# 92MING/Stable-Renderer

Hardware: AMD Instinct MI355X
Metric: frames/sec @512^2, SD1.5 20-step img2img, 8-view overlap (higher is better)
Workload: dtype f16

## Files before the change

### stable-renderer_amd/csrc/igemm.hip

```cpp
#include "sr_common.h"
#ifndef SR_IGEMM_TRACE
#define SR_IGEMM_TRACE 0
#endif
#if SR_IGEMM_TRACE
#define SR_TS(k) do { if (threadIdx.x == 0) ts_[k] = wall_clock64(); } while (0)
#else
#define SR_TS(k) do { } while (0)
#endif
#include <stdlib.h>
#include <type_traits>

namespace {

#define SR_FOLD(p) ((p).row_stats != nullptr || (p).ln_inline != 0)
__device__ __forceinline__ float2 sr_fold_stat(const sr_igemm_args& p, const int m, const int m0) {
  extern __shared__ __attribute__((aligned(16))) char sr_lds_front[];
  if (p.ln_inline) return *(const float2*)(sr_lds_front + 8 * (m - m0));
  return *(const float2*)(p.row_stats + 2 * (int64_t)m);
}

template <typename T, int BM, int BN, int WAVES_M, int WAVES_N, int LDS_AVAIL, bool GEGLU, int VCAP, bool VECPRE>
__device__ __forceinline__ void epilogue_rows_h(const sr_igemm_args& p, f32x4 (&acc)[BN / WAVES_N / 16][BM / WAVES_M / 16], char* smem, const int M,
                                                const int rpb, const int m0, const int n0, const int pm0, const int qn0, const int wv,
                                                const int lane) {
  constexpr int NW = WAVES_M * WAVES_N, TM = BM / WAVES_M / 16, TN = BN / WAVES_N / 16;
  constexpr int WCOLS = BN / WAVES_N, OCOLS = GEGLU ? WCOLS / 2 : WCOLS;
  constexpr int ROWB = OCOLS * 2 + 16;
  constexpr int CPR = OCOLS * 2 / 16, RPI = 64 / CPR;
  constexpr int VEC_B = 2 * BN * 4;
  constexpr int LDS_ROWS = VECPRE ? LDS_AVAIL : LDS_AVAIL - VEC_B;
  constexpr int ACC = TM * TN * 4;
  constexpr auto iters = [](int tmp) { return (tmp * 16 + RPI - 1) / RPI; };
  constexpr auto fits = [](int tmp) { return tmp >= 1 && TM % tmp == 0 && NW * tmp * 16 * ROWB <= LDS_ROWS; };
  constexpr auto pre_ok = [](int tmp) { return ACC + (TM / tmp) * ((tmp * 16 + RPI - 1) / RPI) * 4 + 48 <= VCAP; };
  constexpr auto roll_ok = [](int tmp) { return TM / tmp > 1 && ACC + 2 * ((tmp * 16 + RPI - 1) / RPI) * 4 + 40 <= VCAP; };
  constexpr int T_LDS = fits(TM) ? TM : (fits(TM / 2) ? TM / 2 : 1);
  constexpr int TMP = pre_ok(T_LDS) ? T_LDS : (roll_ok(T_LDS) ? T_LDS : ((T_LDS > 1 && roll_ok(T_LDS / 2) && fits(T_LDS / 2)) ? T_LDS / 2 : ((T_LDS > 1 && roll_ok(1)) ? 1 : T_LDS)));
  constexpr int ROWS = TMP * 16, ITER = iters(TMP), NPASS = TM / TMP;
  constexpr bool PRE = pre_ok(TMP);
  constexpr bool ROLL = !PRE && roll_ok(TMP);
  static_assert(OCOLS % 8 == 0 && NW * 16 * ROWB <= LDS_ROWS, "epilogue staging");
  const int c16 = lane & 15, g4 = lane >> 4;
  const float scale = p.scale;
  const int N = p.N;
  const int ldr = p.rowvec_ld ? p.rowvec_ld : N;
  const int ldo = GEGLU ? (N >> 1) : N;
  float* lvec = (float*)(VECPRE ? smem - VEC_B : smem);
  char* wl = smem + (VECPRE ? 0 : VEC_B) + wv * (ROWS * ROWB);
  const int lr = lane / CPR, lc = lane - lr * CPR;
  const int ncol = (GEGLU ? ((n0 + qn0) >> 1) : (n0 + qn0)) + lc * 8;
  const bool lane_on = lr < RPI && ncol < ldo;
  const int tid = wv * 64 + lane;

  float4 vb = make_float4(0.f, 0.f, 0.f, 0.f), vc = make_float4(0.f, 0.f, 0.f, 0.f);
  if constexpr (!VECPRE) {
    const bool vec_lane = tid < BN / 4 && n0 + tid * 4 < N;
    if (vec_lane) {
      if (p.bias) vb = *(const float4*)(p.bias + n0 + tid * 4);
      if (SR_FOLD(p)) vc = *(const float4*)(p.colsum + n0 + tid * 4);
    }
  }
  uint4 resid[PRE ? NPASS * ITER : 1];
  if constexpr (PRE) {
    if (p.residual) {
#pragma unroll
      for (int ps = 0; ps < NPASS; ++ps)
#pragma unroll
        for (int it = 0; it < ITER; ++it) {
          const int row = it * RPI + lr, m = m0 + pm0 + ps * ROWS + row;
          resid[ps * ITER + it] = make_uint4(0, 0, 0, 0);
          if (lane_on && row < ROWS && m < M) resid[ps * ITER + it] = *(const uint4*)((const _Float16*)p.residual + (int64_t)m * ldo + ncol);
        }
    }
  }
  uint4 rcur[ROLL ? ITER : 1], rnext[ROLL ? ITER : 1];
  auto roll_load = [&](uint4 (&dst)[ROLL ? ITER : 1], int ps) {
#pragma unroll
    for (int it = 0; it < (ROLL ? ITER : 1); ++it) {
      const int row = it * RPI + lr, m = m0 + pm0 + ps * ROWS + row;
      dst[it] = make_uint4(0, 0, 0, 0);
      if (lane_on && row < ROWS && m < M) dst[it] = *(const uint4*)((const _Float16*)p.residual + (int64_t)m * ldo + ncol);
    }
  };
  if constexpr (ROLL) { if (p.residual) roll_load(rcur, 0); }
  __syncthreads();
  if constexpr (!VECPRE) {
    if (tid < BN / 4) { *(float4*)(lvec + tid * 4) = vb; *(float4*)(lvec + BN + tid * 4) = vc; }
    __syncthreads();
  }
#pragma unroll
  for (int ps = 0; ps < NPASS; ++ps) {
#pragma unroll
    for (int t = 0; t < TMP; ++t) {
      const int tm = ps * TMP + t;
      const int m = m0 + pm0 + tm * 16 + c16;
      const int b = (p.rowvec && m < M) ? m / rpb : 0;
      float2 rs = make_float2(1.f, 0.f);
      if (SR_FOLD(p) && m < M) rs = sr_fold_stat(p, m, m0);
#pragma unroll
      for (int tn = 0; tn < TN; ++tn) {
        const int nl = qn0 + tn * 16 + 4 * g4, n = n0 + nl;
        float v[4] = {acc[tn][tm][0] * scale, acc[tn][tm][1] * scale, acc[tn][tm][2] * scale, acc[tn][tm][3] * scale};
        if (n < N) {
          if (SR_FOLD(p)) {
            const float4 cs = *(const float4*)(lvec + BN + nl);
            v[0] = fmaf(rs.x, v[0], rs.y * cs.x); v[1] = fmaf(rs.x, v[1], rs.y * cs.y);
            v[2] = fmaf(rs.x, v[2], rs.y * cs.z); v[3] = fmaf(rs.x, v[3], rs.y * cs.w);
          }
          if (p.bias) { const float4 bv = *(const float4*)(lvec + nl); v[0] += bv.x; v[1] += bv.y; v[2] += bv.z; v[3] += bv.w; }
          if (p.rowvec) { const float4 rv = *(const float4*)(p.rowvec + (int64_t)b * ldr + n); v[0] += rv.x; v[1] += rv.y; v[2] += rv.z; v[3] += rv.w; }
        }
        if (p.act == 1) { for (int r = 0; r < 4; ++r) v[r] = sr_silu_f(v[r]); }
        else if (p.act == 3) { for (int r = 0; r < 4; ++r) v[r] = sr_gelu_f(v[r]); }
        else if (p.act == 4) { for (int r = 0; r < 4; ++r) v[r] = fminf(fmaxf((v[r] + 1.0f) * 0.5f, 0.0f), 1.0f); }
        char* dst = wl + (t * 16 + c16) * ROWB;
        if constexpr (GEGLU) {
          const float o0 = v[0] * sr_gelu_f(v[1]), o1 = v[2] * sr_gelu_f(v[3]);
          h16x2 hv = {(_Float16)o0, (_Float16)o1};
          *(h16x2*)(dst + (tn * 8 + 2 * g4) * 2) = hv;
        } else {
          h16x4 hv = {(_Float16)v[0], (_Float16)v[1], (_Float16)v[2], (_Float16)v[3]};
          *(h16x4*)(dst + (tn * 16 + 4 * g4) * 2) = hv;
        }
      }
    }
    __builtin_amdgcn_s_waitcnt(0xC07F);
    __builtin_amdgcn_wave_barrier();
    if constexpr (ROLL) { if (p.residual && ps + 1 < NPASS) roll_load(rnext, ps + 1); }
#pragma unroll
    for (int it = 0; it < ITER; ++it) {
      const int row = it * RPI + lr, m = m0 + pm0 + ps * ROWS + row;
      if (!(lane_on && row < ROWS && m < M)) continue;
      uint4 raw = *(const uint4*)(wl + row * ROWB + lc * 16);
      const int64_t oi = (int64_t)m * ldo + ncol;
      if (p.residual) {
        const h16x8 rr = PRE ? __builtin_bit_cast(h16x8, resid[PRE ? ps * ITER + it : 0])
                       : ROLL ? __builtin_bit_cast(h16x8, rcur[ROLL ? it : 0]) : *(const h16x8*)((const _Float16*)p.residual + oi);
        h16x8 hv = __builtin_bit_cast(h16x8, raw);
#pragma unroll
        for (int e = 0; e < 8; ++e) hv[e] = (_Float16)((float)hv[e] + (float)rr[e]);
        raw = __builtin_bit_cast(uint4, hv);
      }
      *(uint4*)((_Float16*)p.out + oi) = raw;
    }
    if constexpr (ROLL) {
#pragma unroll
      for (int it = 0; it < ITER; ++it) rcur[it] = rnext[it];
    }
    __builtin_amdgcn_wave_barrier();
  }
}

template <typename T, int BM, int BN, int WAVES_M, int WAVES_N, int LDS_AVAIL, bool BLOCK_SYNC = true, int VCAP = 256, bool VECPRE = false>
__device__ __forceinline__ void epilogue_rows(const sr_igemm_args& p, f32x4 (&acc)[BN / WAVES_N / 16][BM / WAVES_M / 16], char* smem, const int M,
                                              const int rpb, const int m0, const int n0, const int pm0, const int qn0, const int wv,
                                              const int lane) {
  constexpr int NW = WAVES_M * WAVES_N, TM = BM / WAVES_M / 16, TN = BN / WAVES_N / 16;
  const int c16 = lane & 15, g4 = lane >> 4;
  const float scale = p.scale;
  const int N = p.N;
  const int ldr = p.rowvec_ld ? p.rowvec_ld : N;
  {
    const int ldo = (p.act == 2) ? (N >> 1) : N;
    const bool o32 = p.out_f32 || sizeof(T) == 4;
    const int oes = o32 ? 4 : 2;
    if constexpr (sizeof(T) == 2) {
      if (!o32 && (ldo * 2) % 16 == 0) {
        static_assert(BLOCK_SYNC, "the fp16 epilogue synchronises the workgroup itself");
        if (p.act == 2) epilogue_rows_h<T, BM, BN, WAVES_M, WAVES_N, LDS_AVAIL, true, VCAP, VECPRE>(p, acc, smem, M, rpb, m0, n0, pm0, qn0, wv, lane);
        else            epilogue_rows_h<T, BM, BN, WAVES_M, WAVES_N, LDS_AVAIL, false, VCAP, VECPRE>(p, acc, smem, M, rpb, m0, n0, pm0, qn0, wv, lane);
        return;
      }
    }
    if ((ldo * oes) % 16 == 0) {
      constexpr int WCOLS = BN / WAVES_N;
      constexpr int TMP = (NW * (BM / WAVES_M) * (WCOLS * 4 + 16) <= LDS_AVAIL) ? TM : 1;
      const int ocols = (p.act == 2) ? WCOLS / 2 : WCOLS;
      const int rowb = ocols * oes + 16;
      if constexpr (BLOCK_SYNC) __syncthreads();
      char* wl = smem + wv * ((TMP * 16) * rowb);
      const int cpr = ocols * oes / 16;
      const int rpi = 64 / cpr;
      const int lr = lane / cpr, lc = lane - lr * cpr;
      const int ncol0 = (p.act == 2) ? ((n0 + qn0) >> 1) : (n0 + qn0);
      const int epc_o = 16 / oes;
#pragma unroll
     for (int tm0 = 0; tm0 < TM; tm0 += TMP) {
#pragma unroll
      for (int tm = tm0; tm < tm0 + TMP; ++tm) {
        const int m = m0 + pm0 + tm * 16 + c16;
        const int b = (m < M) ? m / rpb : 0;
        float2 rs = make_float2(1.f, 0.f);
        if (SR_FOLD(p) && m < M) rs = sr_fold_stat(p, m, m0);
#pragma unroll
        for (int tn = 0; tn < TN; ++tn) {
          const int n = n0 + qn0 + tn * 16 + 4 * g4;
          float v[4] = {acc[tn][tm][0] * scale, acc[tn][tm][1] * scale, acc[tn][tm][2] * scale, acc[tn][tm][3] * scale};
          if (n < N) {
            if (SR_FOLD(p)) {
              const float4 cs = *(const float4*)(p.colsum + n);
              v[0] = fmaf(rs.x, v[0], rs.y * cs.x); v[1] = fmaf(rs.x, v[1], rs.y * cs.y);
              v[2] = fmaf(rs.x, v[2], rs.y * cs.z); v[3] = fmaf(rs.x, v[3], rs.y * cs.w);
            }
            if (p.bias) { const float4 bv = *(const float4*)(p.bias + n); v[0] += bv.x; v[1] += bv.y; v[2] += bv.z; v[3] += bv.w; }
            if (p.rowvec) { const float4 rv = *(const float4*)(p.rowvec + (int64_t)b * ldr + n); v[0] += rv.x; v[1] += rv.y; v[2] += rv.z; v[3] += rv.w; }
          }
          if (p.act == 1) { for (int r = 0; r < 4; ++r) v[r] = sr_silu_f(v[r]); }
          else if (p.act == 3) { for (int r = 0; r < 4; ++r) v[r] = sr_gelu_f(v[r]); }
          else if (p.act == 4) { for (int r = 0; r < 4; ++r) v[r] = fminf(fmaxf((v[r] + 1.0f) * 0.5f, 0.0f), 1.0f); }
          char* dst = wl + ((tm - tm0) * 16 + c16) * rowb;
          if (p.act == 2) {
            const float o0 = v[0] * sr_gelu_f(v[1]), o1 = v[2] * sr_gelu_f(v[3]);
            const int col = tn * 8 + 2 * g4;
            if (o32) *(float2*)(dst + col * 4) = make_float2(o0, o1);
            else { h16x2 hv = {(_Float16)o0, (_Float16)o1}; *(h16x2*)(dst + col * 2) = hv; }
          } else {
            const int col = tn * 16 + 4 * g4;
            if (o32) *(float4*)(dst + col * 4) = make_float4(v[0], v[1], v[2], v[3]);
            else { h16x4 hv = {(_Float16)v[0], (_Float16)v[1], (_Float16)v[2], (_Float16)v[3]}; *(h16x4*)(dst + col * 2) = hv; }
          }
        }
      }
      __builtin_amdgcn_s_waitcnt(0xC07F);
      __builtin_amdgcn_wave_barrier();
      for (int r0 = 0; r0 < TMP * 16; r0 += rpi) {
        const int row = r0 + lr;
        if (lr >= rpi || row >= TMP * 16) continue;
        const int m = m0 + pm0 + tm0 * 16 + row, ncol = ncol0 + lc * epc_o;
        if (m >= M || ncol >= ldo) continue;
        uint4 raw = *(const uint4*)(wl + row * rowb + lc * 16);
        const int64_t oi = (int64_t)m * ldo + ncol;
        if (p.residual) {
          if constexpr (sizeof(T) == 2) {
            if (o32) {
              float4 f = __builtin_bit_cast(float4, raw);
              const h16x4 r4 = *(const h16x4*)((const _Float16*)p.residual + oi);
              f.x += (float)r4[0]; f.y += (float)r4[1]; f.z += (float)r4[2]; f.w += (float)r4[3];
              raw = __builtin_bit_cast(uint4, f);
            } else {
              const h16x8 rr = *(const h16x8*)((const _Float16*)p.residual + oi);
              h16x8 hv = __builtin_bit_cast(h16x8, raw);
#pragma unroll
              for (int e = 0; e < 8; ++e) hv[e] = (_Float16)((float)hv[e] + (float)rr[e]);
              raw = __builtin_bit_cast(uint4, hv);
            }
          } else {
            float4 f = __builtin_bit_cast(float4, raw);
            const float4 rr = *(const float4*)((const float*)p.residual + oi);
            f.x += rr.x; f.y += rr.y; f.z += rr.z; f.w += rr.w;
            raw = __builtin_bit_cast(uint4, f);
          }
        }
        *(uint4*)((char*)p.out + oi * oes) = raw;
      }
      __builtin_amdgcn_wave_barrier();
     }
      return;
    }
#pragma unroll
    for (int tm = 0; tm < TM; ++tm) {
      const int m = m0 + pm0 + tm * 16 + c16;
      if (m >= M) continue;
      const int b = m / rpb;
#pragma unroll
      for (int tn = 0; tn < TN; ++tn) {
        const int n = n0 + qn0 + tn * 16 + 4 * g4;
        if (n >= N) continue;
        float v[4] = {acc[tn][tm][0] * scale, acc[tn][tm][1] * scale, acc[tn][tm][2] * scale, acc[tn][tm][3] * scale};
        const int nv = (N - n) < 4 ? (N - n) : 4;
        if (SR_FOLD(p)) {
          const float2 rs = sr_fold_stat(p, m, m0);
          for (int r = 0; r < nv; ++r) v[r] = fmaf(rs.x, v[r], rs.y * p.colsum[n + r]);
        }
        if (p.bias) { for (int r = 0; r < nv; ++r) v[r] += p.bias[n + r]; }
        if (p.rowvec) { for (int r = 0; r < nv; ++r) v[r] += p.rowvec[(int64_t)b * ldr + n + r]; }
        if (p.act == 1) { for (int r = 0; r < 4; ++r) v[r] = sr_silu_f(v[r]); }
        else if (p.act == 3) { for (int r = 0; r < 4; ++r) v[r] = sr_gelu_f(v[r]); }
        else if (p.act == 4) { for (int r = 0; r < 4; ++r) v[r] = fminf(fmaxf((v[r] + 1.0f) * 0.5f, 0.0f), 1.0f); }
        if (p.act == 2) {
          float o0 = v[0] * sr_gelu_f(v[1]), o1 = v[2] * sr_gelu_f(v[3]);
          const int64_t oi = (int64_t)m * ldo + (n >> 1);
          if (p.residual) { o0 += sr_load_f((const T*)p.residual + oi); o1 += sr_load_f((const T*)p.residual + oi + 1); }
          if (p.out_f32) { float* o = (float*)p.out + oi; o[0] = o0; o[1] = o1; }
          else { T* o = (T*)p.out + oi; sr_store_f(o, o0); sr_store_f(o + 1, o1); }
// ... 568 lines not shown
  if (ntail > SR_IGEMM_SPLIT_COUNTERS) as.split_counters = nullptr;
  hipLaunchKernelGGL(ks, dim3(ntail, S), dim3(256), lds, st, as, M, Ho, Wo, NTv, ntail, tile0);
  if (!as.split_counters) {
    constexpr int FR = (BM / 32) * (BN / 32);
    hipLaunchKernelGGL((splitk_reduce_kernel<T, BM, BN>), dim3(ntail * FR), dim3(256), 0, st, a, M, Ho * Wo, S, NTv, ntail, tile0);
  }
  SR_CHECK_LAUNCH("sr_igemm(split-K)");
  return SR_OK;
}

__global__ __launch_bounds__(512, 1) void conv3p_kernel(const sr_igemm_args p, const int M, const int NT, const int nwg) {
  using T = _Float16;
  extern __shared__ __attribute__((aligned(16))) char smem_all[];
  char* const smem = smem_all + 8 * 256;
  constexpr int BM = 256, BN = 320, WAVES_M = 4, WAVES_N = 2, TM = 4, TN = 10;
  constexpr int APITCH = 80, ABYTES = 32768, BBYTES = BN * 64, BOFF = 2 * ABYTES, LDS_TOTAL = BOFF + 4 * BBYTES;
  const int tid = threadIdx.x, lane = tid & 63;
  const int wv = __builtin_amdgcn_readfirstlane(tid >> 6);
  if (p.prefetch)
    sr_prefetch_touch(p.prefetch, p.prefetch_bytes, (int64_t)blockIdx.x * 512 + tid, (int64_t)gridDim.x * 512,
                      __builtin_amdgcn_readfirstlane(sr_lds_addr(smem_all) + wv * 256));
  const int wg = sr_xcd_remap(blockIdx.x, nwg);
  const int mt = wg / NT, nt = wg - mt * NT;
  const int m0 = mt * BM, n0 = nt * BN;
  const int H = p.H, W = p.W, C1 = p.C1, rpb = H * W;
  const int ipt = rpb >= 256 ? 1 : 256 / rpb;
  const int Ri = rpb >= 256 ? 256 / W : H;
  const int PW = W + 2, HPI = (Ri + 2) * PW, HR = ipt * HPI;
  const int b0 = m0 / rpb, y0 = (m0 - b0 * rpb) / W;

  unsigned aoffg[4];
#pragma unroll
  for (int i = 0; i < 4; ++i) {
    const int u = (wv * 4 + i) * 64 + lane;
    const int hrow = u / 5, ch = u - hrow * 5;
    const int img = hrow / HPI, rem = hrow - img * HPI, hr = rem / PW, hc = rem - hr * PW;
    const int y = y0 + hr - 1, x = hc - 1, b = b0 + img;
    const bool ok = ch < 4 && hrow < HR && y >= 0 && y < H && x >= 0 && x < W && b < p.B;
    aoffg[i] = ok ? (unsigned)(((((int64_t)b * H + y) * W + x) * C1) * 2 + ch * 16) : 0xFFFFFFFFu;
    if (!ok) {
      *(uint4*)(smem + (wv * 4 + i) * 1024 + lane * 16) = make_uint4(0, 0, 0, 0);
      *(uint4*)(smem + ABYTES + (wv * 4 + i) * 1024 + lane * 16) = make_uint4(0, 0, 0, 0);
    }
  }
  asm volatile("s_waitcnt lgkmcnt(0)" ::: "memory");
  const int lrow = lane >> 2;
  const int lchunk = (0x1320 >> (4 * ((lane & 3) ^ ((lrow >> 2) & 3)))) & 3;
  const unsigned wlane = (unsigned)(lrow * 9 * C1 * 2 + lchunk * 16);
  const unsigned ldsA = __builtin_amdgcn_readfirstlane(sr_lds_addr(smem)), ldsB = ldsA + BOFF;
  int ac = 0;
  auto issueA = [&](int buf, int i) {
    if (aoffg[i] != 0xFFFFFFFFu) sr_glds16_asm_saddr(aoffg[i], (const char*)p.a + (int64_t)ac * 64, ldsA + buf * ABYTES + (wv * 4 + i) * 1024);
  };
  int lc = 0, lt = 0;
  auto issueB = [&](int slot) {
    const char* wb = (const char*)p.w + ((int64_t)n0 * 9 * C1 + lt * C1 + lc * 32) * 2;
#pragma unroll
    for (int i = 0; i < 3; ++i) {
      const int gi = (i * 8 + wv) < 20 ? (i * 8 + wv) : 19;
      sr_glds16_asm_saddr(wlane, wb + (int64_t)gi * 16 * 9 * C1 * 2, ldsB + slot * BBYTES + gi * 1024);
    }
    if (++lt == 9) { lt = 0; ++lc; }
  };

  const int c16 = lane & 15, g4 = lane >> 4;
  const int wm = wv >> 1, wn = wv & 1;
  const int pm0 = wm * 64, qn0 = wn * 160;
  int aoff0, adel[TM];
  {
    const int riw = Ri * W;
    auto hrow_of = [&](int pi) { const int img = pi / riw, q = pi - img * riw, r = q / W, cx = q - r * W; return img * HPI + r * PW + cx; };
    aoff0 = hrow_of(pm0 + c16) * APITCH + g4 * 16;
#pragma unroll
    for (int j = 0; j < TM; ++j) adel[j] = __builtin_amdgcn_readfirstlane((hrow_of(pm0 + j * 16) - hrow_of(pm0)) * APITCH);
  }
  const int foffB = qn0 * 64 + c16 * 64 + ((((c16 >> 2) & 3) ^ ((0x2130 >> (4 * g4)) & 3)) << 4);
  const int pw80 = PW * APITCH;

  f32x4 acc[TN][TM];
#pragma unroll
  for (int a = 0; a < TN; ++a)
#pragma unroll
    for (int b = 0; b < TM; ++b) acc[a][b] = f32x4{0.f, 0.f, 0.f, 0.f};

  const int NC = C1 / 32;
  {
    const unsigned m0k = sr_m0_save();
#pragma unroll
    for (int i = 0; i < 4; ++i) issueA(0, i);
    ac = 1;
    issueB(0); issueB(1); issueB(2);
    sr_m0_restore(m0k);
  }
  int s = 0;
  auto chunk = [&](auto lastc, const int c) {
    constexpr bool LASTC = decltype(lastc)::value;
    auto step = [&](auto tc) {
      constexpr int t = decltype(tc)::value;
      constexpr int nx = LASTC ? (t <= 6 ? 6 : (t == 7 ? 3 : 0))
                               : 6 + (t >= 1 && t <= 4) + (t >= 2 && t <= 5) + (t >= 3 && t <= 6);
      asm volatile("s_waitcnt vmcnt(%0)" ::"n"(nx) : "memory");
      __builtin_amdgcn_s_barrier();
      const char* Bq = smem + BOFF + (s & 3) * BBYTES + foffB;
      int to = (t / 3) * pw80 + (t % 3) * APITCH + (c & 1) * ABYTES;
      asm volatile("" : "+s"(to));
      uint4 xf[TM], wf[TN];
#pragma unroll
      for (int j = 0; j < TM; ++j) xf[j] = *(const uint4*)(smem + aoff0 + (adel[j] + to));
#pragma unroll
      for (int tn = 0; tn < TN; ++tn) wf[tn] = *(const uint4*)(Bq + tn * 1024);
      if (!LASTC || t < 6) {
        const unsigned m0k = sr_m0_save();
        issueB((s + 3) & 3);
        if constexpr (!LASTC) { if (t < 4) issueA((c + 1) & 1, t); if (t == 3) ++ac; }
        sr_m0_restore(m0k);
      }
#pragma unroll
      for (int tn = 0; tn < TN; ++tn)
#pragma unroll
        for (int tm = 0; tm < TM; ++tm) sr_mma(acc[tn][tm], wf[tn], xf[tm], T());
      ++s;
    };
    step(std::integral_constant<int, 0>{}); step(std::integral_constant<int, 1>{}); step(std::integral_constant<int, 2>{});
    step(std::integral_constant<int, 3>{}); step(std::integral_constant<int, 4>{}); step(std::integral_constant<int, 5>{});
    step(std::integral_constant<int, 6>{}); step(std::integral_constant<int, 7>{}); step(std::integral_constant<int, 8>{});
  };
  for (int c = 0; c < NC - 1; ++c) chunk(std::false_type{}, c);
  chunk(std::true_type{}, NC - 1);

  epilogue_rows<T, BM, BN, WAVES_M, WAVES_N, LDS_TOTAL>(p, acc, smem, M, rpb, m0, n0, pm0, qn0, wv, lane);
}

static bool conv3p_ok(const sr_igemm_args& a, int M) {
  if (a.dtype != SR_F16 || a.KH != 3 || a.stride != 1 || a.upsample || a.C2 || a.transpose_out || a.row_stats || a.ln_inline || a.pad_br) return false;
  if (a.C1 % 64 || a.N % 320 || M % 256 || a.act == 2) return false;
  const int rpb = a.H * a.W;
  if (a.W < 8 || 256 % a.W) { if (!(rpb < 256 && 256 % rpb == 0)) return false; }
  if (rpb >= 256 ? (rpb % 256 != 0 || 256 % a.W != 0) : (256 % rpb != 0)) return false;
  const int ipt = rpb >= 256 ? 1 : 256 / rpb, Ri = rpb >= 256 ? 256 / a.W : a.H;
  if ((int64_t)a.B * rpb * a.C1 * 2 >= 0xFFFFFFFFLL) return false;
  return ipt * (Ri + 2) * (a.W + 2) * 80 <= 32768;
}

static int launch_conv3p(const sr_igemm_args& a, int M, hipStream_t st) {
  constexpr int lds = 2 * 32768 + 4 * 320 * 64 + 8 * 256;
  const int NT = a.N / 320, nwg = (M / 256) * NT;
  static bool attr_set = false;
  if (!attr_set) { (void)hipFuncSetAttribute((const void*)conv3p_kernel, hipFuncAttributeMaxDynamicSharedMemorySize, lds); attr_set = true; }
  hipLaunchKernelGGL(conv3p_kernel, dim3(nwg), dim3(512), lds, st, a, M, NT, nwg);
  SR_CHECK_LAUNCH("sr_igemm(conv3p)");
  return SR_OK;
}

static inline int plan_split(int64_t tiles, int KT, int slots, double t_k, int64_t tile_ws_bytes, int64_t ws_bytes, int* tile0, int forceS = 0) {
  const int64_t full = tiles / slots, tail = tiles - full * slots;
  *tile0 = (int)(full * slots);
  if (tail == 0) return 1;
  if (forceS > 0)
    return (KT / forceS >= 4 && (int64_t)forceS * tail * tile_ws_bytes <= ws_bytes) ? forceS : -1;
  if (const char* fs = getenv("SR_SPLIT_S")) {
    const int S = atoi(fs);
    if (S >= 1 && KT / S >= 4 && (int64_t)S * tail * tile_ws_bytes <= ws_bytes) return S;
  }
  double best = (double)KT * t_k;
  int bestS = 1;
  for (int S = 2; S <= 16; ++S) {
    if (KT / S < 8 || (int64_t)S * tail * tile_ws_bytes > ws_bytes) break;
    const int64_t rounds = (tail * S + slots - 1) / slots;
    const double t = (double)rounds * ((KT + S - 1) / S) * t_k + (double)(2 * S * tail * tile_ws_bytes) / 4.0e6 + 14.0;
    if (t < best * 0.9) { best = t; bestS = S; }
  }
  return bestS;
}

template <typename T, bool TRANS>
int dispatch(const sr_igemm_args& a, int M, int Ho, int Wo, hipStream_t st) {
  const int n128 = (a.N + 127) / 128, n64 = (a.N + 63) / 64;
  const int64_t wg_128x128 = (int64_t)((M + 127) / 128) * n128;
  const bool waste128 = (n128 * 128 - a.N) * 8 > a.N;
  const char* fenv = getenv("SR_IGEMM_TILE");
  const int force = fenv ? atoi(fenv) : a.tile;
  static const bool split_off = getenv("SR_SPLITK") && atoi(getenv("SR_SPLITK")) == 0;
  const int KT = a.KH * a.KH * ((a.C1 + a.C2) / (int)(128 / sizeof(T)));
  const int forceS = a.split > 1 ? a.split : 0;
  const bool can_split = !TRANS && !split_off && a.split >= 0 && a.workspace && a.act != 2 && a.N % 4 == 0 && !a.ln_inline;
  const bool may_split = can_split && KT >= 32;
  const bool deep_split = can_split && KT >= 8 && (force == 14 || force == 15);
  if (forceS && !((may_split && (force == 2 || force == 3)) || deep_split))
    SR_FAIL(SR_ERR_INVALID, "sr_igemm: split = %d needs tile 2 / 3 (K >= 32 steps) or 14 / 15 (K >= 8 steps), a workspace, no GEGLU / transposed output", a.split);
  if constexpr (!TRANS) {
    if (deep_split && forceS) {
      int tile0 = 0;
      const int64_t tiles = force == 15 ? wg_128x128 : (int64_t)((M + 127) / 128) * n64;
      const int S = plan_split(tiles, KT, 256, 1.0, 128 * (force == 15 ? 128 : 64) * 4, a.workspace_bytes, &tile0, forceS);
      if (S < 0) SR_FAIL(SR_ERR_INVALID, "sr_igemm: split = %d does not fit this shape (K steps %d, workspace %lld B)", a.split, KT, (long long)a.workspace_bytes);
      if (S > 1) return force == 15 ? launch_split<T, 128, 128, 4>(a, M, Ho, Wo, tile0, S, st) : launch_split<T, 128, 64, 6>(a, M, Ho, Wo, tile0, S, st);
      SR_FAIL(SR_ERR_INVALID, "sr_igemm: split = %d: nothing to split (whole rounds of workgroups only)", a.split);
    }
    if (may_split && (force == 2 || force == 3)) {
      int tile0 = 0;
      if (force == 2) {
        const int S = plan_split(wg_128x128, KT, 512, 1.2, 128 * 128 * 4, a.workspace_bytes, &tile0, forceS);
        if (S < 0) SR_FAIL(SR_ERR_INVALID, "sr_igemm: split = %d does not fit this shape (K steps %d, workspace %lld B)", a.split, KT, (long long)a.workspace_bytes);
        if (S > 1) return launch_split<T, 128, 128>(a, M, Ho, Wo, tile0, S, st);
      } else {
        const int S = plan_split((int64_t)((M + 127) / 128) * n64, KT, 768, 0.93, 128 * 64 * 4, a.workspace_bytes, &tile0, forceS);
        if (S < 0) SR_FAIL(SR_ERR_INVALID, "sr_igemm: split = %d does not fit this shape (K steps %d, workspace %lld B)", a.split, KT, (long long)a.workspace_bytes);
        if (S > 1) return launch_split<T, 128, 64>(a, M, Ho, Wo, tile0, S, st);
      }
      if (forceS) SR_FAIL(SR_ERR_INVALID, "sr_igemm: split = %d: nothing to split (whole rounds of workgroups only)", a.split);
    }
  }
  if (force == 2) return launch_ln<T, 128, 128, 2, 2, 2, TRANS>(a, M, Ho, Wo, st);
  if (force == 3) return launch_ln<T, 128, 64, 2, 2, 2, TRANS>(a, M, Ho, Wo, st);
  if (force == 4) return launch_ln<T, 64, 64, 2, 2, 2, TRANS>(a, M, Ho, Wo, st);
  if (force == 13) return launch_ln<T, 64, 64, 2, 2, 8, TRANS>(a, M, Ho, Wo, st);
  if (force == 14) return launch_ln<T, 128, 64, 2, 2, 6, TRANS>(a, M, Ho, Wo, st);
  if (force == 15) return launch_ln<T, 128, 128, 2, 2, 4, TRANS>(a, M, Ho, Wo, st);
  if (force == 8) {
    if constexpr (!TRANS && sizeof(T) == 2) { if (conv3p_ok(a, M)) return launch_conv3p(a, M, st); }
    SR_FAIL(SR_ERR_INVALID, "sr_igemm: tile 8 (patch-stationary 3x3) needs fp16, KH=3, stride 1, one source, N %% 320 == 0, "
                            "256-pixel tiles of whole rows / images (H=%d W=%d M=%d N=%d)", a.H, a.W, M, a.N);
  }
  if constexpr (!TRANS && sizeof(T) == 2) {
    if ((force >= 5 && force <= 7) && a.N % 320) SR_FAIL(SR_ERR_INVALID, "sr_igemm: tile %d (256x320) needs N %% 320 == 0, N=%d", force, a.N);
    if (force == 6) return launch<T, 256, 320, 4, 2, 4, TRANS, 64>(a, M, Ho, Wo, st);
    if (force == 9) {
      if (a.N % 160) SR_FAIL(SR_ERR_INVALID, "sr_igemm: tile 9 (128x160) needs N %% 160 == 0, N=%d", a.N);
      return launch_ln<T, 128, 160, 4, 2, 2, TRANS, 128, 0, 4>(a, M, Ho, Wo, st);
    }
    if (force == 10) {
      if (a.N % 320) SR_FAIL(SR_ERR_INVALID, "sr_igemm: tile 10 (128x320) needs N %% 320 == 0, N=%d", a.N);
      return launch_ln<T, 128, 320, 2, 4, 2, TRANS, 64, 0, 4>(a, M, Ho, Wo, st);
    }
    if (force == 11) return launch_ln<T, 128, 128, 4, 2, 2, TRANS, 128, 0, 4>(a, M, Ho, Wo, st);
    if (force == 12) return launch_ln<T, 256, 128, 4, 2, 2, TRANS, 64, 0, 4>(a, M, Ho, Wo, st);
    if (force == 7 || (force == 0 && a.N % 320 == 0 && (int64_t)((M + 255) / 256) * (a.N / 320) < 256 &&
                       (int64_t)((M + 127) / 128) * (a.N / 320) >= 256))
      return launch_ln<T, 128, 320, 2, 4, 2, TRANS>(a, M, Ho, Wo, st);

    if (force == 5 || (force == 0 && a.N % 320 == 0 && (int64_t)((M + 255) / 256) * (a.N / 320) >= 256))
      return launch_ln<T, 256, 320, 4, 2, 2, TRANS, 128, 2>(a, M, Ho, Wo, st);
  } else {
    if (force >= 5 && force <= 12) SR_FAIL(SR_ERR_INVALID, "sr_igemm: tile %d is fp16, non-transposed only", force);
  }
  const int64_t wg_256x128 = (int64_t)((M + 255) / 256) * n128;
  const bool big = !waste128 && wg_256x128 >= 512;
  if constexpr (!TRANS) {
    if (force == 0 && may_split && !big) {
      int tile0 = 0;
      if (!waste128) {
        const int S = plan_split(wg_128x128, KT, 512, 1.2, 128 * 128 * 4, a.workspace_bytes, &tile0);
        if (S > 1) return launch_split<T, 128, 128>(a, M, Ho, Wo, tile0, S, st);
      } else {
        const int S = plan_split((int64_t)((M + 127) / 128) * n64, KT, 768, 0.93, 128 * 64 * 4, a.workspace_bytes, &tile0);
        if (S > 1) return launch_split<T, 128, 64>(a, M, Ho, Wo, tile0, S, st);
      }
    }
  }
  if (force == 1 || (force == 0 && big && !a.ln_inline))
    return launch<T, 256, 128, 4, 2, 3, TRANS, 128, 1>(a, M, Ho, Wo, st);
  if (!waste128 && wg_128x128 >= 192 && !(a.KH == 1 && wg_128x128 <= 768)) return launch_ln<T, 128, 128, 2, 2, 2, TRANS>(a, M, Ho, Wo, st);
  const int64_t wg_128x64 = (int64_t)((M + 127) / 128) * n64;
  if (wg_128x64 >= 192) return launch_ln<T, 128, 64, 2, 2, 2, TRANS>(a, M, Ho, Wo, st);
  if ((int64_t)((M + 63) / 64) * n64 <= 256 && KT >= 4) return launch_ln<T, 64, 64, 2, 2, 8, TRANS>(a, M, Ho, Wo, st);
  return launch_ln<T, 64, 64, 2, 2, 2, TRANS>(a, M, Ho, Wo, st);
}

}

static int igemm_check(const sr_igemm_args* a, int* M_, int* Ho_, int* Wo_) {
  if (!a || !a->a || !a->w || !a->out || !a->zero_page) SR_FAIL(SR_ERR_INVALID, "sr_igemm: null pointer");
  const int ke = a->dtype == SR_F16 ? 64 : 32;
  if (a->dtype != SR_F16 && a->dtype != SR_F32) SR_FAIL(SR_ERR_INVALID, "sr_igemm: bad dtype %d", a->dtype);
  if (a->C1 <= 0 || a->C1 % ke || a->C2 % ke || a->C2 < 0) SR_FAIL(SR_ERR_INVALID, "sr_igemm: C1=%d C2=%d must be multiples of %d", a->C1, a->C2, ke);
  if (a->C2 > 0 && !a->a2) SR_FAIL(SR_ERR_INVALID, "sr_igemm: C2>0 without a2");
  if (a->KH != 1 && a->KH != 3) SR_FAIL(SR_ERR_INVALID, "sr_igemm: KH=%d", a->KH);
  if (a->stride != 1 && a->stride != 2) SR_FAIL(SR_ERR_INVALID, "sr_igemm: stride=%d", a->stride);
  if (a->upsample && a->stride != 1) SR_FAIL(SR_ERR_INVALID, "sr_igemm: upsample with stride");
  if (a->pad_br && (a->KH != 3 || a->upsample)) SR_FAIL(SR_ERR_INVALID, "sr_igemm: pad_br is for 3x3 convs without upsample");
  if (a->N <= 0 || a->B <= 0 || a->H <= 0 || a->W <= 0) SR_FAIL(SR_ERR_INVALID, "sr_igemm: bad sizes");
  if (a->act == 2 && (a->N % 4 || a->transpose_out)) SR_FAIL(SR_ERR_INVALID, "sr_igemm: GEGLU needs N%%4==0");
  if (a->row_stats && !a->colsum) SR_FAIL(SR_ERR_INVALID, "sr_igemm: row_stats without colsum");
  if (a->ln_inline && (a->row_stats || !a->colsum)) SR_FAIL(SR_ERR_INVALID, "sr_igemm: ln_inline takes colsum and no row_stats");
  if ((a->row_stats || a->ln_inline) && (a->KH != 1 || a->stride != 1 || a->upsample || a->C2)) SR_FAIL(SR_ERR_INVALID, "sr_igemm: folded LayerNorm is for 1x1 single-source layers");
  if (a->tile < 0 || a->tile > 15 || a->split < -1 || a->split == 1 || a->split > 16) SR_FAIL(SR_ERR_INVALID, "sr_igemm: tile=%d split=%d", a->tile, a->split);
  if (a->tile_order != 0 && a->tile_order != 1) SR_FAIL(SR_ERR_INVALID, "sr_igemm: tile_order=%d (0 rows first, 1 columns first)", a->tile_order);
  int Ho, Wo;
  if (a->upsample && ((a->up_h > 0) != (a->up_w > 0))) SR_FAIL(SR_ERR_INVALID, "sr_igemm: up_h / up_w go together");
  if (!a->upsample && (a->up_h || a->up_w)) SR_FAIL(SR_ERR_INVALID, "sr_igemm: up_h / up_w without upsample");
  if (a->upsample) { Ho = a->up_h > 0 ? a->up_h : 2 * a->H; Wo = a->up_w > 0 ? a->up_w : 2 * a->W; }
  else if (a->stride == 2) {
    const int ptot = a->pad_br ? a->KH / 2 : 2 * (a->KH / 2);
    Ho = (a->H + ptot - a->KH) / 2 + 1; Wo = (a->W + ptot - a->KH) / 2 + 1;
  }
  else { Ho = a->H; Wo = a->W; }
  const int64_t M64 = (int64_t)a->B * Ho * Wo;
  if (M64 > 0x7fffffffLL / 2) SR_FAIL(SR_ERR_INVALID, "sr_igemm: M too large");
  auto off = [](const void* p, uintptr_t al) { return ((uintptr_t)p & (al - 1)) != 0; };
  if (off(a->a, 16) || off(a->a2, 16) || off(a->w, 16) || off(a->zero_page, 16) || off(a->bias, 16) || off(a->colsum, 16) ||
      off(a->rowvec, 16) || off(a->residual, 16) || off(a->out, 16) || off(a->workspace, 16))
    SR_FAIL(SR_ERR_INVALID, "sr_igemm: a / a2 / w / zero_page / bias / colsum / rowvec / residual / out / workspace must be 16-byte aligned");
  if (off(a->row_stats, 8) || off(a->split_counters, 4) || off(a->prefetch, 4))
    SR_FAIL(SR_ERR_INVALID, "sr_igemm: row_stats must be 8-byte, split_counters / prefetch 4-byte aligned");
  if (a->rowvec && a->rowvec_ld % 4 && a->N % 4 == 0) SR_FAIL(SR_ERR_INVALID, "sr_igemm: rowvec_ld=%d must be a multiple of 4 floats", a->rowvec_ld);
  if (a->transpose_out && a->ldt < Ho * Wo) SR_FAIL(SR_ERR_INVALID, "sr_igemm: ldt < pixels per batch");
  *M_ = (int)M64; *Ho_ = Ho; *Wo_ = Wo;
  return SR_OK;
}

extern "C" int sr_igemm(const sr_igemm_args* a, void* stream) {
  int M, Ho, Wo;
  const int rc = igemm_check(a, &M, &Ho, &Wo);
  if (rc != SR_OK) return rc;
  hipStream_t st = sr_stream(stream);
  if (a->dtype == SR_F16) {
    return a->transpose_out ? dispatch<_Float16, true>(*a, M, Ho, Wo, st) : dispatch<_Float16, false>(*a, M, Ho, Wo, st);
  }
  return a->transpose_out ? dispatch<float, true>(*a, M, Ho, Wo, st) : dispatch<float, false>(*a, M, Ho, Wo, st);
}

template <typename T>
static int group_launch(int tile, const sr_igemm_args* const* as, const int* Ms, const int* Hos, const int* Wos, int n, hipStream_t st) {
  switch (tile) {
    case 2: return launch_group<T, 128, 128, 2, 2, 2>(as, Ms, Hos, Wos, n, st);
    case 3: return launch_group<T, 128, 64, 2, 2, 2>(as, Ms, Hos, Wos, n, st);
    case 4: return launch_group<T, 64, 64, 2, 2, 2>(as, Ms, Hos, Wos, n, st);
    case 13: return launch_group<T, 64, 64, 2, 2, 8>(as, Ms, Hos, Wos, n, st);
    case 14: return launch_group<T, 128, 64, 2, 2, 6>(as, Ms, Hos, Wos, n, st);
    case 15: return launch_group<T, 128, 128, 2, 2, 4>(as, Ms, Hos, Wos, n, st);
    default: break;
  }
  if constexpr (sizeof(T) == 2) {
    if (tile == 9) return launch_group<T, 128, 160, 4, 2, 2, 128, 0, 4>(as, Ms, Hos, Wos, n, st);
    if (tile == 10) return launch_group<T, 128, 320, 2, 4, 2, 64, 0, 4>(as, Ms, Hos, Wos, n, st);
  }
  return -100;
}

extern "C" int sr_igemm_group(const sr_igemm_args* const* args, int32_t n, void* stream) {
  if (!args || n < 1 || n > SR_IGEMM_GROUP_MAX) SR_FAIL(SR_ERR_INVALID, "sr_igemm_group: 1..%d problems", SR_IGEMM_GROUP_MAX);
  int M[SR_IGEMM_GROUP_MAX], Ho[SR_IGEMM_GROUP_MAX], Wo[SR_IGEMM_GROUP_MAX];
  bool one = n > 1;
  for (int i = 0; i < n; ++i) {
    const int rc = igemm_check(args[i], &M[i], &Ho[i], &Wo[i]);
    if (rc != SR_OK) return rc;
    const sr_igemm_args* a = args[i];
    one = one && a->dtype == args[0]->dtype && a->tile == args[0]->tile && a->tile != 0 && !a->transpose_out && a->split == -1;
    if (a->tile == 9) one = one && a->N % 160 == 0;
    if (a->tile == 10) one = one && a->N % 320 == 0;
  }
  hipStream_t st = sr_stream(stream);
  if (one) {
    const int rc = args[0]->dtype == SR_F16 ? group_launch<_Float16>(args[0]->tile, args, M, Ho, Wo, n, st)
                                            : group_launch<float>(args[0]->tile, args, M, Ho, Wo, n, st);
    if (rc != -100) return rc;
  }
  for (int i = 0; i < n; ++i) {
    const int rc = sr_igemm(args[i], stream);
    if (rc != SR_OK) return rc;
  }
  return SR_OK;
}
```

Baseline: 21.58.

## Add patch-stationary 3x3 conv kernels with 16x16 halo tiles for N not multiple of 320

After: 21.56 (median of 2 runs). No clear change (-0.1%).

```diff
diff --git a/stable-renderer_amd/csrc/igemm.hip b/stable-renderer_amd/csrc/igemm.hip
--- a/stable-renderer_amd/csrc/igemm.hip
+++ b/stable-renderer_amd/csrc/igemm.hip
@@ -19,10 +19,11 @@
   return *(const float2*)(p.row_stats + 2 * (int64_t)m);
 }
 
-template <typename T, int BM, int BN, int WAVES_M, int WAVES_N, int LDS_AVAIL, bool GEGLU, int VCAP, bool VECPRE>
+struct sr_rows_linear { __device__ __forceinline__ int operator()(const int m0, const int l) const { return m0 + l; } };
+template <typename T, int BM, int BN, int WAVES_M, int WAVES_N, int LDS_AVAIL, bool GEGLU, int VCAP, bool VECPRE, typename RM = sr_rows_linear>
 __device__ __forceinline__ void epilogue_rows_h(const sr_igemm_args& p, f32x4 (&acc)[BN / WAVES_N / 16][BM / WAVES_M / 16], char* smem, const int M,
                                                 const int rpb, const int m0, const int n0, const int pm0, const int qn0, const int wv,
-                                                const int lane) {
+                                                const int lane, const RM rm = RM()) {
   constexpr int NW = WAVES_M * WAVES_N, TM = BM / WAVES_M / 16, TN = BN / WAVES_N / 16;
   constexpr int WCOLS = BN / WAVES_N, OCOLS = GEGLU ? WCOLS / 2 : WCOLS;
   constexpr int ROWB = OCOLS * 2 + 16;
@@ -67,7 +68,7 @@
       for (int ps = 0; ps < NPASS; ++ps)
 #pragma unroll
         for (int it = 0; it < ITER; ++it) {
-          const int row = it * RPI + lr, m = m0 + pm0 + ps * ROWS + row;
+          const int row = it * RPI + lr, m = rm(m0, pm0 + ps * ROWS + row);
           resid[ps * ITER + it] = make_uint4(0, 0, 0, 0);
           if (lane_on && row < ROWS && m < M) resid[ps * ITER + it] = *(const uint4*)((const _Float16*)p.residual + (int64_t)m * ldo + ncol);
         }
@@ -77,7 +78,7 @@
   auto roll_load = [&](uint4 (&dst)[ROLL ? ITER : 1], int ps) {
 #pragma unroll
     for (int it = 0; it < (ROLL ? ITER : 1); ++it) {
-      const int row = it * RPI + lr, m = m0 + pm0 + ps * ROWS + row;
+      const int row = it * RPI + lr, m = rm(m0, pm0 + ps * ROWS + row);
       dst[it] = make_uint4(0, 0, 0, 0);
       if (lane_on && row < ROWS && m < M) dst[it] = *(const uint4*)((const _Float16*)p.residual + (int64_t)m * ldo + ncol);
     }
@@ -93,7 +94,7 @@
 #pragma unroll
     for (int t = 0; t < TMP; ++t) {
       const int tm = ps * TMP + t;
-      const int m = m0 + pm0 + tm * 16 + c16;
+      const int m = rm(m0, pm0 + tm * 16 + c16);
       const int b = (p.rowvec && m < M) ? m / rpb : 0;
       float2 rs = make_float2(1.f, 0.f);
       if (SR_FOLD(p) && m < M) rs = sr_fold_stat(p, m, m0);
@@ -129,7 +130,7 @@
     if constexpr (ROLL) { if (p.residual && ps + 1 < NPASS) roll_load(rnext, ps + 1); }
 #pragma unroll
     for (int it = 0; it < ITER; ++it) {
-      const int row = it * RPI + lr, m = m0 + pm0 + ps * ROWS + row;
+      const int row = it * RPI + lr, m = rm(m0, pm0 + ps * ROWS + row);
       if (!(lane_on && row < ROWS && m < M)) continue;
       uint4 raw = *(const uint4*)(wl + row * ROWB + lc * 16);
       const int64_t oi = (int64_t)m * ldo + ncol;
@@ -1004,6 +1005,277 @@
   return SR_OK;
 }
 
+struct sr_rows_patch16 {
+  int W;
+  __device__ __forceinline__ int operator()(const int m0, const int l) const { return m0 + (l >> 4) * W + (l & 15); }
+};
+
+template <int BN>
+__global__ __launch_bounds__(512, 1) void conv3w_kernel(const sr_igemm_args p, const int M, const int NT, const int nwg) {
+  using T = _Float16;
+  extern __shared__ __attribute__((aligned(16))) char smem_all[];
+  char* const smem = smem_all + 8 * 256;
+  constexpr int BM = 256, WAVES_M = 4, WAVES_N = 2, TM = 4, TN = BN / WAVES_N / 16, PB = BN / 128;
+  constexpr int TP = 16, PW = TP + 2, HR = PW * PW;
+  constexpr int APITCH = 80, ABYTES = 32768, BBYTES = BN * 64, BOFF = 2 * ABYTES, LDS_TOTAL = BOFF + 4 * BBYTES;
+  const int tid = threadIdx.x, lane = tid & 63;
+  const int wv = __builtin_amdgcn_readfirstlane(tid >> 6);
+  const unsigned ldsZ = __builtin_amdgcn_readfirstlane(sr_lds_addr(smem_all) + wv * 256);
+  if (p.prefetch)
+    sr_prefetch_touch(p.prefetch, p.prefetch_bytes, (int64_t)blockIdx.x * 512 + tid, (int64_t)gridDim.x * 512, ldsZ);
+  const int wg = sr_xcd_remap(blockIdx.x, nwg);
+  const int mt = wg / NT, nt = wg - mt * NT;
+  const int n0 = nt * BN;
+  const int H = p.H, W = p.W, C1 = p.C1, rpb = H * W;
+  const int tpr = W / TP, tpi = (H / TP) * tpr;
+  const int b0 = mt / tpi, pr = mt - b0 * tpi, y0 = (pr / tpr) * TP, x0 = (pr - (pr / tpr) * tpr) * TP;
+  const int mbase = (b0 * H + y0) * W + x0;
+
+  unsigned aoffg[4];
+  bool apiece[4];
+#pragma unroll
+  for (int i = 0; i < 4; ++i) {
+    const int u = (wv * 4 + i) * 64 + lane;
+    const int hrow = u / 5, ch = u - hrow * 5;
+    const int hr = hrow / PW, hc = hrow - hr * PW;
+    const int y = y0 + hr - 1, x = x0 + hc - 1;
+    const bool ok = ch < 4 && hrow < HR && y >= 0 && y < H && x >= 0 && x < W;
+    aoffg[i] = ok ? (unsigned)(((((int64_t)b0 * H + y) * W + x) * C1) * 2 + ch * 16) : 0xFFFFFFFFu;
+    apiece[i] = __builtin_amdgcn_readfirstlane(__ballot(ok) != 0ull ? 1 : 0) != 0;
+    if (!ok) {
+      *(uint4*)(smem + (wv * 4 + i) * 1024 + lane * 16) = make_uint4(0, 0, 0, 0);
+      *(uint4*)(smem + ABYTES + (wv * 4 + i) * 1024 + lane * 16) = make_uint4(0, 0, 0, 0);
+    }
+  }
+  asm volatile("s_waitcnt lgkmcnt(0)" ::: "memory");
+  const int lrow = lane >> 2;
+  const int lchunk = (0x1320 >> (4 * ((lane & 3) ^ ((lrow >> 2) & 3)))) & 3;
+  const unsigned wlane = (unsigned)(lrow * 9 * C1 * 2 + lchunk * 16);
+  const unsigned ldsA = __builtin_amdgcn_readfirstlane(sr_lds_addr(smem)), ldsB = ldsA + BOFF;
+  int ac = 0;
+  auto issueA = [&](int buf, int i) {
+    const char* ab = (const char*)p.a + (int64_t)ac * 64;
+    if (apiece[i]) {
+      if (aoffg[i] != 0xFFFFFFFFu) sr_glds16_asm_saddr(aoffg[i], ab, ldsA + buf * ABYTES + (wv * 4 + i) * 1024);
+    } else {
+      asm volatile("s_mov_b32 m0, %2\n\ts_nop 0\n\tglobal_load_lds_dword %0, %1" ::"v"((unsigned)(lane * 4)), "s"(ab), "s"(ldsZ) : "memory");
+    }
+  };
+  int lc = 0, lt = 0;
+  auto issueB = [&](int slot) {
+    const char* wb = (const char*)p.w + ((int64_t)n0 * 9 * C1 + lt * C1 + lc * 32) * 2;
+#pragma unroll
+    for (int i = 0; i < PB; ++i) {
+      const int gi = i * 8 + wv;
+      sr_glds16_asm_saddr(wlane, wb + (int64_t)gi * 16 * 9 * C1 * 2, ldsB + slot * BBYTES + gi * 1024);
+    }
+    if (++lt == 9) { lt = 0; ++lc; }
+  };
+
+  const int c16 = lane & 15, g4 = lane >> 4;
+  const int wm = wv >> 1, wn = wv & 1;
+  const int pm0 = wm * 64, qn0 = wn * (BN / 2);
+  const int aoff0 = ((wm * 4) * PW + c16) * APITCH + g4 * 16;
+  const int foffB = qn0 * 64 + c16 * 64 + ((((c16 >> 2) & 3) ^ ((0x2130 >> (4 * g4)) & 3)) << 4);
+  constexpr int pw80 = PW * APITCH;
+
+  f32x4 acc[TN][TM];
+#pragma unroll
+  for (int a = 0; a < TN; ++a)
+#pragma unroll
+    for (int b = 0; b < TM; ++b) acc[a][b] = f32x4{0.f, 0.f, 0.f, 0.f};
+
+  const int NC = C1 / 32;
+  {
+    const unsigned m0k = sr_m0_save();
+#pragma unroll
+    for (int i = 0; i < 4; ++i) issueA(0, i);
+    ac = 1;
+    issueB(0); issueB(1); issueB(2);
+    sr_m0_restore(m0k);
+  }
+  int s = 0;
+  auto chunk = [&](auto lastc, const int c) {
+    constexpr bool LASTC = decltype(lastc)::value;
+    auto step = [&](auto tc) {
+      constexpr int t = decltype(tc)::value;
+      constexpr int nx = LASTC ? (t <= 6 ? 2 * PB : (t == 7 ? PB : 0))
+                               : 2 * PB + (t >= 1 && t <= 4) + (t >= 2 && t <= 5) + (t >= 3 && t <= 6);
+      asm volatile("s_waitcnt vmcnt(%0)" ::"n"(nx) : "memory");
+      __builtin_amdgcn_s_barrier();
+      const char* Bq = smem + BOFF + (s & 3) * BBYTES + foffB;
+      int to = (t / 3) * pw80 + (t % 3) * APITCH + (c & 1) * ABYTES;
+      asm volatile("" : "+s"(to));
+      uint4 xf[TM], wf[TN];
+#pragma unroll
+      for (int j = 0; j < TM; ++j) xf[j] = *(const uint4*)(smem + aoff0 + (j * pw80 + to));
+#pragma unroll
+      for (int tn = 0; tn < TN; ++tn) wf[tn] = *(const uint4*)(Bq + tn * 1024);
+      if (!LASTC || t < 6) {
+        const unsigned m0k = sr_m0_save();
+        issueB((s + 3) & 3);
+        if constexpr (!LASTC) { if (t < 4) issueA((c + 1) & 1, t); if (t == 3) ++ac; }
+        sr_m0_restore(m0k);
+      }
+#pragma unroll
+      for (int tn = 0; tn < TN; ++tn)
+#pragma unroll
+        for (int tm = 0; tm < TM; ++tm) sr_mma(acc[tn][tm], wf[tn], xf[tm], T());
+      ++s;
+    };
+    step(std::integral_constant<int, 0>{}); step(std::integral_constant<int, 1>{}); step(std::integral_constant<int, 2>{});
+    step(std::integral_constant<int, 3>{}); step(std::integral_constant<int, 4>{}); step(std::integral_constant<int, 5>{});
+    step(std::integral_constant<int, 6>{}); step(std::integral_constant<int, 7>{}); step(std::integral_constant<int, 8>{});
+  };
+  for (int c = 0; c < NC - 1; ++c) chunk(std::false_type{}, c);
+  chunk(std::true_type{}, NC - 1);
+
+  epilogue_rows_h<T, BM, BN, WAVES_M, WAVES_N, LDS_TOTAL, false, 256, false, sr_rows_patch16>(p, acc, smem, M, rpb, mbase, n0, pm0, qn0, wv, lane,
+                                                                                             sr_rows_patch16{W});
+}
+
+__global__ __launch_bounds__(512, 4) void conv3n_kernel(const sr_igemm_args p, const int M, const int nwg) {
+  using T = _Float16;
+  extern __shared__ __attribute__((aligned(16))) char smem_all[];
+  char* const smem = smem_all + 8 * 256;
+  constexpr int TP = 16, PW = TP + 2, HR = PW * PW, APITCH = 80, NPIECE = 26, ABYTES = NPIECE * 1024, WBYTES = 9 * 1024, BOFF = 2 * ABYTES;
+  static_assert(HR * APITCH <= ABYTES, "halo buffer");
+  const int tid = threadIdx.x, lane = tid & 63;
+  const int wv = __builtin_amdgcn_readfirstlane(tid >> 6);
+  if (p.prefetch)
+    sr_prefetch_touch(p.prefetch, p.prefetch_bytes, (int64_t)blockIdx.x * 512 + tid, (int64_t)gridDim.x * 512,
+                      __builtin_amdgcn_readfirstlane(sr_lds_addr(smem_all) + wv * 256));
+  const int mt = sr_xcd_remap(blockIdx.x, nwg);
+  const int H = p.H, W = p.W, C1 = p.C1;
+  const int tpr = W / TP, tpi = (H / TP) * tpr;
+  const int b0 = mt / tpi, pr = mt - b0 * tpi, y0 = (pr / tpr) * TP, x0 = (pr - (pr / tpr) * tpr) * TP;
+  const int mbase = (b0 * H + y0) * W + x0;
+
+  unsigned aoffg[4];
+#pragma unroll
+  for (int i = 0; i < 4; ++i) {
+    const int k = wv * 4 + i, u = k * 64 + lane;
+    const int hrow = u / 5, ch = u - hrow * 5;
+    const int hr = hrow / PW, hc = hrow - hr * PW;
+    const int y = y0 + hr - 1, x = x0 + hc - 1;
+    const bool ok = k < NPIECE && ch < 4 && hrow < HR && y >= 0 && y < H && x >= 0 && x < W;
+    aoffg[i] = ok ? (unsigned)(((((int64_t)b0 * H + y) * W + x) * C1) * 2 + ch * 16) : 0xFFFFFFFFu;
+    if (!ok && k < NPIECE) {
+      *(uint4*)(smem + k * 1024 + lane * 16) = make_uint4(0, 0, 0, 0);
+      *(uint4*)(smem + ABYTES + k * 1024 + lane * 16) = make_uint4(0, 0, 0, 0);
+    }
+  }
+  asm volatile("s_waitcnt lgkmcnt(0)" ::: "memory");
+  const int lrow = lane >> 2;
+  const int lchunk = (0x1320 >> (4 * ((lane & 3) ^ ((lrow >> 2) & 3)))) & 3;
+  const unsigned wlane = (unsigned)(lrow * 9 * C1 * 2 + lchunk * 16);
+  const unsigned ldsA = __builtin_amdgcn_readfirstlane(sr_lds_addr(smem)), ldsB = ldsA + BOFF;
+  auto issue = [&](const int c) {
+    const int buf = c & 1;
+    const unsigned m0k = sr_m0_save();
+#pragma unroll
+    for (int i = 0; i < 4; ++i)
+      if (aoffg[i] != 0xFFFFFFFFu) sr_glds16_asm_saddr(aoffg[i], (const char*)p.a + (int64_t)c * 64, ldsA + buf * ABYTES + (wv * 4 + i) * 1024);
+    for (int t = wv; t < 9; t += 8)
+      sr_glds16_asm_saddr(wlane, (const char*)p.w + ((int64_t)t * C1 + c * 32) * 2, ldsB + buf * WBYTES + t * 1024);
+    sr_m0_restore(m0k);
+  };
+
+  const int c16 = lane & 15, g4 = lane >> 4;
+  const int pm0 = wv * 32;
+  const int aoff0 = ((wv * 2) * PW + c16) * APITCH + g4 * 16;
+  const int foffB = c16 * 64 + ((((c16 >> 2) & 3) ^ ((0x2130 >> (4 * g4)) & 3)) << 4);
+  constexpr int pw80 = PW * APITCH;
+  f32x4 acc[2] = {f32x4{0.f, 0.f, 0.f, 0.f}, f32x4{0.f, 0.f, 0.f, 0.f}};
+
+  const int NC = C1 / 32;
+  issue(0);
+  for (int c = 0; c < NC; ++c) {
+    asm volatile("s_waitcnt vmcnt(0)" ::: "memory");
+    __builtin_amdgcn_s_barrier();
+    if (c + 1 < NC) issue(c + 1);
+    const char* Aq = smem + (c & 1) * ABYTES + aoff0;
+    const char* Bq = smem + BOFF + (c & 1) * WBYTES + foffB;
+#pragma unroll
+    for (int t = 0; t < 9; ++t) {
+      const uint4 wf = *(const uint4*)(Bq + t * 1024);
+#pragma unroll
+      for (int j = 0; j < 2; ++j) {
+        const uint4 xf = *(const uint4*)(Aq + (j + t / 3) * pw80 + (t % 3) * APITCH);
+        sr_mma(acc[j], wf, xf, T());
+      }
+    }
+  }
+
+  const int N = p.N, n = 4 * g4;
+  if (n >= N) return;
+  const int nv = (N - n) < 4 ? (N - n) : 4;
+  const int ldr = p.rowvec_ld ? p.rowvec_ld : N;
+#pragma unroll
+  for (int j = 0; j < 2; ++j) {
+    const int l = pm0 + j * 16 + c16;
+    const int m = mbase + (l >> 4) * W + (l & 15);
+    float v[4] = {acc[j][0] * p.scale, acc[j][1] * p.scale, acc[j][2] * p.scale, acc[j][3] * p.scale};
+    if (p.bias) { for (int r = 0; r < nv; ++r) v[r] += p.bias[n + r]; }
+    if (p.rowvec) { for (int r = 0; r < nv; ++r) v[r] += p.rowvec[(int64_t)b0 * ldr + n + r]; }
+    if (p.act == 1) { for (int r = 0; r < 4; ++r) v[r] = sr_silu_f(v[r]); }
+    else if (p.act == 3) { for (int r = 0; r < 4; ++r) v[r] = sr_gelu_f(v[r]); }
+    else if (p.act == 4) { for (int r = 0; r < 4; ++r) v[r] = fminf(fmaxf((v[r] + 1.0f) * 0.5f, 0.0f), 1.0f); }
+    const int64_t oi = (int64_t)m * N + n;
+    for (int r = 0; r < nv; ++r) {
+      float o = v[r];
+      if (p.residual) o += sr_load_f((const T*)p.residual + oi + r);
+      if (p.out_f32) ((float*)p.out)[oi + r] = o; else sr_store_f((T*)p.out + oi + r, o);
+    }
+  }
+}
+
+static const char* conv3w_why_not(const sr_igemm_args& a) {
+  if (a.dtype != SR_F16) return "fp16";
+  if (a.KH != 3 || a.stride != 1 || a.upsample) return "KH = 3, stride 1, no upsample";
+  if (a.C2) return "one source (C2 == 0)";
+  if (a.transpose_out) return "a row-major output";
+  if (a.row_stats || a.ln_inline || a.pad_br) return "no row_stats / ln_inline / pad_br";
+  if (a.act == 2) return "act != 2";
+  if (a.C1 % 64) return "C1 % 64 == 0";
+  if (a.N > 8 && a.N % 128) return "N % 128 == 0 or N <= 8";
+  if (a.N > 8 && a.out_f32) return "an fp16 output (fp32 only at N <= 8)";
+  if (a.H % 16 || a.W % 16) return "H % 16 == 0 and W % 16 == 0";
+  if ((int64_t)a.B * a.H * a.W * a.C1 * 2 >= 0xFFFFFFFFLL) return "an input below 4 GiB (32-bit source offsets)";
+  return nullptr;
+}
+static bool conv3w_ok(const sr_igemm_args& a) { return conv3w_why_not(a) == nullptr; }
+
+static bool conv3w_auto(const sr_igemm_args& a, int M) {
+  if (!conv3w_ok(a) || a.N % 320 == 0) return false;
+  if (a.N <= 8) return M / 256 >= 512;
+  return (int64_t)(M / 256) * (a.N / 128) >= 512;
+}
+
+template <int BN>
+static int launch_conv3w_bn(const sr_igemm_args& a, int M, hipStream_t st) {
+  constexpr int lds = 2 * 32768 + 4 * BN * 64 + 8 * 256;
+  const int NT = a.N / BN, nwg = (M / 256) * NT;
+  static bool attr_set = false;
+  if (!attr_set) { (void)hipFuncSetAttribute((const void*)conv3w_kernel<BN>, hipFuncAttributeMaxDynamicSharedMemorySize, lds); attr_set = true; }
+  hipLaunchKernelGGL(conv3w_kernel<BN>, dim3(nwg), dim3(512), lds, st, a, M, NT, nwg);
+  SR_CHECK_LAUNCH("sr_igemm(conv3w)");
+  return SR_OK;
+}
+static int launch_conv3n(const sr_igemm_args& a, int M, hipStream_t st) {
+  constexpr int lds = 8 * 256 + 2 * 26 * 1024 + 2 * 9 * 1024;
+  const int nwg = M / 256;
+  static bool attr_set = false;
+  if (!attr_set) { (void)hipFuncSetAttribute((const void*)conv3n_kernel, hipFuncAttributeMaxDynamicSharedMemorySize, lds); attr_set = true; }
+  hipLaunchKernelGGL(conv3n_kernel, dim3(nwg), dim3(512), lds, st, a, M, nwg);
+  SR_CHECK_LAUNCH("sr_igemm(conv3n)");
+  return SR_OK;
+}
+static int launch_conv3w(const sr_igemm_args& a, int M, hipStream_t st) {
+  if (a.N <= 8) return launch_conv3n(a, M, st);
+  return a.N % 256 == 0 ? launch_conv3w_bn<256>(a, M, st) : launch_conv3w_bn<128>(a, M, st);
+}
+
 static inline int plan_split(int64_t tiles, int KT, int slots, double t_k, int64_t tile_ws_bytes, int64_t ws_bytes, int* tile0, int forceS = 0) {
   const int64_t full = tiles / slots, tail = tiles - full * slots;
   *tile0 = (int)(full * slots);
@@ -1074,7 +1346,12 @@
     SR_FAIL(SR_ERR_INVALID, "sr_igemm: tile 8 (patch-stationary 3x3) needs fp16, KH=3, stride 1, one source, N %% 320 == 0, "
                             "256-pixel tiles of whole rows / images (H=%d W=%d M=%d N=%d)", a.H, a.W, M, a.N);
   }
+  if (force == 16) {
+    if constexpr (!TRANS && sizeof(T) == 2) { if (conv3w_ok(a)) return launch_conv3w(a, M, st); }
+    SR_FAIL(SR_ERR_INVALID, "sr_igemm: tile 16 (patch-stationary 3x3, 16x16 patches) needs %s (H=%d W=%d C1=%d N=%d)", conv3w_why_not(a), a.H, a.W, a.C1, a.N);
+  }
   if constexpr (!TRANS && sizeof(T) == 2) {
+    if (force == 0 && conv3w_auto(a, M)) return launch_conv3w(a, M, st);
     if ((force >= 5 && force <= 7) && a.N % 320) SR_FAIL(SR_ERR_INVALID, "sr_igemm: tile %d (256x320) needs N %% 320 == 0, N=%d", force, a.N);
     if (force == 6) return launch<T, 256, 320, 4, 2, 4, TRANS, 64>(a, M, Ho, Wo, st);
     if (force == 9) {
@@ -1136,7 +1413,7 @@
   if (a->row_stats && !a->colsum) SR_FAIL(SR_ERR_INVALID, "sr_igemm: row_stats without colsum");
   if (a->ln_inline && (a->row_stats || !a->colsum)) SR_FAIL(SR_ERR_INVALID, "sr_igemm: ln_inline takes colsum and no row_stats");
   if ((a->row_stats || a->ln_inline) && (a->KH != 1 || a->stride != 1 || a->upsample || a->C2)) SR_FAIL(SR_ERR_INVALID, "sr_igemm: folded LayerNorm is for 1x1 single-source layers");
-  if (a->tile < 0 || a->tile > 15 || a->split < -1 || a->split == 1 || a->split > 16) SR_FAIL(SR_ERR_INVALID, "sr_igemm: tile=%d split=%d", a->tile, a->split);
+  if (a->tile < 0 || a->tile > 16 || a->split < -1 || a->split == 1 || a->split > 16) SR_FAIL(SR_ERR_INVALID, "sr_igemm: tile=%d split=%d", a->tile, a->split);
   if (a->tile_order != 0 && a->tile_order != 1) SR_FAIL(SR_ERR_INVALID, "sr_igemm: tile_order=%d (0 rows first, 1 columns first)", a->tile_order);
   int Ho, Wo;
   if (a->upsample && ((a->up_h > 0) != (a->up_w > 0))) SR_FAIL(SR_ERR_INVALID, "sr_igemm: up_h / up_w go together");
```
